# viodotcom/ppca_rs

Hardware: AMD Instinct MI355X
Metric: EM iters/sec (and samples/sec/iter) at N=10M d=256 k=10, 30% masked (higher is better)
Workload: dtype f64

## Files before the change

ppca_rs_amd/csrc/ppca_em9.hip:

```cpp
#include <cstdlib>

#include "ppca_device.hpp"

namespace ppca {

constexpr int E9_QW = 7;
constexpr int E9_F = 50;
constexpr int E9_HEAD = 6;
constexpr int E9_POISON = 100000;
constexpr int E9_EMIN = -900, E9_EMAX = 1000;
constexpr int E9_FLUSH_GROUPS = 100;
constexpr int E9_X_AUX = 2;
constexpr int E9_Q_AUX = 0;
constexpr int E9_LAC = 4;
constexpr int E9_HEAVY_BUDGET = 8;
constexpr int E9_GS_PAD = 18;
constexpr int E9_P4A_AHEAD = 1;

#ifdef PPCA_PHASE_TIMING
#define E9_FINE(i) { __builtin_amdgcn_sched_barrier(0); long long tn = clock64(); tfine[i] += tn - tfl; tfl = tn; __builtin_amdgcn_sched_barrier(0); }
#else
#define E9_FINE(i)
#endif

__device__ unsigned long long e9_counters[4];

template <int K>
struct Cfg9 {
    using c = Cfg<K>;
    static constexpr int KP = c::KP, NTP = c::NTP, B = c::B, DP = c::DP, XS = c::XS, CS = c::CS;
    static constexpr int NC = KP + K + 1;
    static constexpr int NCT = (NC + 15) / 16;
    static constexpr int NCOL = 16 * NCT;
    static constexpr int NCGB = (K + 3) / 4;
    static constexpr int NCL = NCGB < 2 ? NCGB : 2;
    static constexpr int PADC = K == 10 ? 14 : E9_GS_PAD;
    static constexpr int GS = 16 * NTP + PADC;
    static constexpr int WS = GS;
    static constexpr int NCP = NC;
    static constexpr int PLANE_BYTES = E9_QW * 2 * NCP * 16;
    static constexpr int OFF_X = 0;
    static constexpr int OFF_G = OFF_X + B * XS;
    static constexpr int OFF_W = OFF_G;
    static constexpr int OFF_M = OFF_G + 2 * B * GS;
    static constexpr int OFF_MB = OFF_M + 2 * B * 4;
    static constexpr int OFF_S = OFF_MB + DP * 2;
    static constexpr int OFF_L = OFF_S + 2 * B;
    static constexpr int OFF_P0 = OFF_L + 6 * B;
    static constexpr int OFF_P1 = OFF_P0 + PLANE_BYTES / 8;
    static constexpr int OFF_E = OFF_P1 + PLANE_BYTES / 8;
    static constexpr int OFF_BAR = OFF_E + NCOL / 2 + 4;
    static constexpr int OFF_K = OFF_BAR + 4;
    static constexpr int OFF_EB = OFF_K + 4;
    static constexpr int OFF_XT = OFF_EB + NCOL;
    static constexpr int OFF_CL = OFF_XT + 2 * B * 4;
    static constexpr int LDS_DOUBLES = OFF_CL + 2 * 16 * NCL * 32;
    static constexpr int p1slot(int a) { return a < PADC - K ? 16 * NTP + K + a : KP + (a - (PADC - K)); }
    static_assert(K - (PADC - K) <= 16 * NTP - KP, "free slots of a row hold the second partial of b");
    static_assert(NCOL / 2 <= 64, "one back wave digitises NCOL / 2 (column, chunk) items");
    static_assert(LDS_DOUBLES * 8 <= 160 * 1024, "LDS budget");
};

__device__ __forceinline__ void role_barrier(unsigned *ctr, unsigned &target, int lane) {
    asm volatile("s_waitcnt lgkmcnt(0)" ::: "memory");
    target += 4;
    if (lane == 0) __hip_atomic_fetch_add(ctr, 1u, __ATOMIC_RELAXED, __HIP_MEMORY_SCOPE_WORKGROUP);
    for (;;) {
        const unsigned seen = __builtin_amdgcn_readfirstlane(__hip_atomic_load(ctr, __ATOMIC_RELAXED, __HIP_MEMORY_SCOPE_WORKGROUP));
        if ((int)(seen - target) >= 0) break;
        __builtin_amdgcn_s_sleep(1);
    }
    asm volatile("" ::: "memory");
}
__device__ __forceinline__ void wait_counter(const unsigned *ctr, unsigned need) {
    for (;;) {
        const unsigned seen = __builtin_amdgcn_readfirstlane(__hip_atomic_load(ctr, __ATOMIC_RELAXED, __HIP_MEMORY_SCOPE_WORKGROUP));
        if ((int)(seen - need) >= 0) break;
        __builtin_amdgcn_s_sleep(1);
    }
    asm volatile("" ::: "memory");
}


template <int K, bool GATHER, bool WEIGHTED>
__global__ __launch_bounds__(512) void em9_kernel(PassArgs p) {
    using cfg = Cfg9<K>;
    constexpr int KP = cfg::KP, NTP = cfg::NTP, B = cfg::B, XS = cfg::XS, CS = cfg::CS, GS = cfg::GS,
                  WS = cfg::WS, NC = cfg::NC, NCT = cfg::NCT, NCOL = cfg::NCOL, NCP = cfg::NCP;
    constexpr int NF = 4;
    constexpr int RPW = B / NF;
    constexpr int DPS = cfg::DP / 2;
    constexpr int RT = 16 / NF;
    constexpr int DW = cfg::DP / NF;
    constexpr int QW = E9_QW;
    static_assert(NTP <= NF, "int8 Gram: one front wave per packed-column tile");
    static_assert(QS == 8, "digit grouping assumes 8 slices");
    extern __shared__ __attribute__((aligned(16))) double sm[];
    double *Xs = sm + cfg::OFF_X;
    double *Gs = sm + cfg::OFF_G;
    double *Ws = sm + cfg::OFF_W;
    unsigned long long *Ms = reinterpret_cast<unsigned long long *>(sm + cfg::OFF_M);
    unsigned *Mb = reinterpret_cast<unsigned *>(sm + cfg::OFF_MB);
    double *xxs = sm + cfg::OFF_S;
    double *scl = sm + cfg::OFF_L;
    int *Ex = reinterpret_cast<int *>(sm + cfg::OFF_E);
    unsigned *ctr = reinterpret_cast<unsigned *>(sm + cfg::OFF_BAR);
    unsigned *fbar = ctr, *bbar = ctr + 1, *digdone = ctr + 2, *vstamp = ctr + 3, *wready = ctr + 4, *itdone = ctr + 5, *cbar = ctr + 6;

    if (p.qflag) {
        int unsafe = 0;
#pragma unroll
        for (int t = 0; t < NTP; ++t) unsafe |= p.qflag[t];
        if (unsafe) return;
    }
    const int tid = threadIdx.x, lane_entry = tid & 63;
    const int wave8 = __builtin_amdgcn_readfirstlane(tid >> 6);
    const bool front = wave8 < NF;
    const int wave = wave8 & (NF - 1);
    const int d = p.d;
    const int64_t n = p.n_dev ? (int64_t)*p.n_dev : p.n;
    const double *mC = p.model + MODEL_HDR;
    const double *mMean = mC + (int64_t)d * K;
    const double s2_k = p.model[1], lnsig_k = p.model[2];

    constexpr bool PAIRS = K >= 2;
    constexpr int L_DEV = 0, L_LLK = L_DEV + B, L_W = L_DEV + 2 * B, L_NE = L_DEV + 3 * B, L_PM = L_DEV + 4 * B, L_PX = L_DEV + 5 * B;
    for (int idx = tid; idx < L_DEV + 6 * B; idx += 512) scl[idx] = (idx >= L_PM && idx < L_PX) ? 1.0 : 0.0;
    for (int idx = tid; idx < cfg::DP * 4; idx += 512) Mb[idx] = 0u;
    {
        constexpr int NCL = cfg::NCL, NCGB = cfg::NCGB;
        for (int idx = tid; idx < 2 * 16 * NCL * 32; idx += 512) {
            const int e = idx & 31, blk = idx >> 5, c = blk % NCL, hq = blk / NCL;
            sm[cfg::OFF_CL + idx] = p.cpb[(hq * NCGB + c) * 32 + e];
        }
    }
    if (tid < 8) ctr[tid] = 0u;
    if (tid < 4) Ex[NCOL + tid] = 0;
    if (tid < NCOL) sm[cfg::OFF_EB + tid] = 0.0;
    if (tid == 0) {
        sm[cfg::OFF_K] = s2_k;
        sm[cfg::OFF_K + 1] = 1.0 / s2_k;
        sm[cfg::OFF_K + 2] = lnsig_k;
    }

    const int64_t ntiles = (n + B - 1) / B;
    const int64_t tiles_per_wg = (ntiles + gridDim.x - 1) / gridDim.x;
    const int64_t tile_begin = (int64_t)blockIdx.x * tiles_per_wg;
    const int64_t tile_end = tile_begin + tiles_per_wg < ntiles ? tile_begin + tiles_per_wg : ntiles;
#ifdef PPCA_PHASE_TIMING
    long long tfine[16] = {0, 0, 0, 0, 0, 0, 0, 0, 0, 0, 0, 0, 0, 0, 0, 0};
    long long tfl = clock64();
#endif
    __syncthreads();

    if (!front) {
        typedef double acc_t;
        acc_t accM[RT][NCT][4];
#pragma unroll
        for (int r = 0; r < RT; ++r)
#pragma unroll
            for (int t = 0; t < NCT; ++t)
#pragma unroll
                for (int q = 0; q < 4; ++q) accM[r][t][q] = (acc_t)0;
        unsigned bbar_target = 0u;
        unsigned attempt = 0u;
        int pending = 0;
        int have_scale = 0, flushed = 0, groups = 0;
        int n_rescale = 0, n_flush = 0;
        int hbudget = E9_HEAVY_BUDGET;
        double *ebs = sm + cfg::OFF_EB;
        int rows_win = 0;
        unsigned char *smb = reinterpret_cast<unsigned char *>(sm);
        constexpr int P0_BYTES = cfg::OFF_P0 * 8, PG_BYTES = cfg::OFF_P1 * 8;
        StatsLayout L(d, K);
        double *out = p.part + (int64_t)blockIdx.x * L.len;

        const double *Wcur = Ws;
        auto wsrc = [&](int c) { return c < KP ? c : 16 * NTP + (c - KP); };

        auto digitise = [&](int lane, int dst_bytes, auto heavy_tag, unsigned heavy) -> bool {
            constexpr bool HEAVY = decltype(heavy_tag)::value;
            asm volatile("" : "+v"(lane));
            const bool active = lane < NCOL / 2;
            const int it = (NCOL / 2) * wave + (active ? lane : 0);
            const int c = it >> 1, chunk = it & 1;
            const unsigned hmine = HEAVY ? (heavy >> (16 * chunk)) & 0xFFFFu : 0u;
            const bool cvalid = c < NC;
            const int src = cvalid ? wsrc(c) : 0;
            const int E = Ex[c];
            const bool poisoned = E > 5000;
            const double qsc = __hiloint2double((1023 + E9_F - (poisoned ? 0 : E)) << 20, 0);
            const double magic = __hiloint2double(0x43388080, (int)0x80808080);
            unsigned bad = 0u;
            unsigned pl[QW][4];
            const double *wsrcp = Wcur + (16 * chunk) * WS + src;
#pragma unroll
            for (int g4 = 0; g4 < 4; ++g4) {
                unsigned wlo[4], whi[4];
#pragma unroll
                for (int j = 0; j < 4; ++j) {
                    const double wv = wsrcp[(4 * g4 + j) * WS];
                    const bool take = HEAVY ? cvalid && !((hmine >> (4 * g4 + j)) & 1u) : cvalid;
                    const double v = __builtin_fma(take ? wv : 0.0, qsc, magic);
                    const unsigned lo = (unsigned)__double2loint(v) ^ 0x80808080u;
                    const unsigned hi = (unsigned)__double2hiint(v) ^ 0x43388080u;
                    bad |= hi;
                    const int top = __builtin_amdgcn_sbfe((int)hi, 16, 4);
                    wlo[j] = lo;
                    whi[j] = __builtin_amdgcn_perm((unsigned)top, hi, 0x0C040100u);
                }
                auto tr4 = [&](const unsigned *w, unsigned *o0, unsigned *o1, unsigned *o2, unsigned *o3) {
                    const unsigned t0 = __builtin_amdgcn_perm(w[1], w[0], 0x05010400u), t1 = __builtin_amdgcn_perm(w[1], w[0], 0x07030602u);
                    const unsigned u0 = __builtin_amdgcn_perm(w[3], w[2], 0x05010400u), u1 = __builtin_amdgcn_perm(w[3], w[2], 0x07030602u);
                    *o0 = __builtin_amdgcn_perm(u0, t0, 0x05040100u);
                    *o1 = __builtin_amdgcn_perm(u0, t0, 0x07060302u);
                    *o2 = __builtin_amdgcn_perm(u1, t1, 0x05040100u);
                    if (o3) *o3 = __builtin_amdgcn_perm(u1, t1, 0x07060302u);
                };
                tr4(wlo, &pl[0][g4], &pl[1][g4], &pl[2][g4], &pl[3][g4]);
                tr4(whi, &pl[4][g4], &pl[5][g4], &pl[6][g4], nullptr);
                __builtin_amdgcn_sched_barrier(0);
            }
            if (active && cvalid) {
                unsigned char *wq = smb + dst_bytes;
#pragma unroll
                for (int sl = 0; sl < QW; ++sl)
                    *reinterpret_cast<i4_t *>(wq + ((sl * 2 + chunk) * NCP + c) * 16) =
                        i4_t{(int)pl[sl][0], (int)pl[sl][1], (int)pl[sl][2], (int)pl[sl][3]};
            }
            const bool mine = active && cvalid && !poisoned && (bad >> 20) != 0u;
            return __builtin_amdgcn_ballot_w64(mine) != 0ull;
        };

        auto rescale = [&](int lane, bool robust) {
            asm volatile("" : "+v"(lane));
            const bool active = lane < NCOL / 2;
            const int it = (NCOL / 2) * wave + (active ? lane : 0);
            const int c = it >> 1, chunk = it & 1;
            const bool cvalid = c < NC;
            const int src = cvalid ? wsrc(c) : 0;
            double m = 0.0;
            bool fin = true;
            if (!robust) {
#pragma unroll
                for (int j = 0; j < 16; ++j) {
                    const double av = __builtin_fabs(cvalid ? Wcur[(16 * chunk + j) * WS + src] : 0.0);
                    fin = fin && (av < __builtin_inf());
                    m = __builtin_fmax(m, av);
                }
            } else {
                const int hm = p.heavy_max;
                double cand = 0.0, mx = 0.0;
                for (int j = 0; j < 16; ++j) {
                    const double av = __builtin_fabs(cvalid ? Wcur[(16 * chunk + j) * WS + src] : 0.0);
                    fin = fin && (av < __builtin_inf());
                    mx = __builtin_fmax(mx, av);
                    int above = 0;
                    for (int i = 0; i < 32; ++i) above += __builtin_fabs(cvalid ? Wcur[i * WS + src] : 0.0) > av ? 1 : 0;
                    if (above >= hm) cand = __builtin_fmax(cand, av);
                }
                cand = __builtin_fmax(cand, dpp_f64<0xB1, 0xF>(cand));
                mx = __builtin_fmax(mx, dpp_f64<0xB1, 0xF>(mx));
                m = cand > 0.0 ? cand : mx;
            }
            m = __builtin_fmax(m, dpp_f64<0xB1, 0xF>(m));
            const int finw = __builtin_amdgcn_update_dpp(0, fin ? 1 : 0, 0xB1, 0xF, 0xF, true);
            fin = fin && finw != 0;
            const int Eold = have_scale ? Ex[c] : E9_EMIN;
            int Enew = Eold;
            if (m > 0.0) {
                int e = __builtin_amdgcn_frexp_exp(m) + E9_HEAD;
                e = e < E9_EMIN ? E9_EMIN : e;
                Enew = e > Eold ? e : Eold;
            }
            if (!fin || Enew > E9_EMAX) Enew = E9_POISON;
            if (Eold > 5000) Enew = Eold;
            if (active && chunk == 0) Ex[c] = Enew;
        };

        int *hvw = Ex + NCOL;
        auto heavy_bits = [&](int lane) {
            asm volatile("" : "+v"(lane));
            const bool active = lane < NCOL / 2;
            const int it = (NCOL / 2) * wave + (active ? lane : 0);
            const int c = it >> 1, chunk = it & 1;
            const bool cvalid = c < NC;
            const int src = cvalid ? wsrc(c) : 0;
            const int E = Ex[c];
            const bool live = active && cvalid && E <= 5000;
            const double qsc = __hiloint2double((1023 + E9_F - (live ? E : 0)) << 20, 0);
            const double magic = __hiloint2double(0x43388080, (int)0x80808080);
            unsigned bits = 0u, nogo = 0u;
            for (int j = 0; j < 16; ++j) {
                const double wv = live ? Wcur[(16 * chunk + j) * WS + src] : 0.0;
                const double v = __builtin_fma(wv, qsc, magic);
                const unsigned hi = (unsigned)__double2hiint(v) ^ 0x43388080u;
                if ((hi >> 20) != 0u) {
                    bits |= 1u << (16 * chunk + j);
                    if (!(__builtin_fabs(wv) < __builtin_inf()) || __builtin_amdgcn_frexp_exp(wv) + E9_F - E > 1000) nogo = 1u;
                }
            }
            if (bits) __hip_atomic_fetch_or(reinterpret_cast<unsigned *>(hvw), bits, __ATOMIC_RELAXED, __HIP_MEMORY_SCOPE_WORKGROUP);
            if (nogo) __hip_atomic_fetch_or(reinterpret_cast<unsigned *>(hvw + 1), 1u, __ATOMIC_RELAXED, __HIP_MEMORY_SCOPE_WORKGROUP);
        };
        auto heavy_add = [&](int lane, unsigned hv, int slot) {
            asm volatile("" : "+v"(lane));
            const int l15 = lane & 15, l4 = lane >> 4;
            unsigned mw[RT][4];
#pragma unroll
            for (int r = 0; r < RT; ++r)
#pragma unroll
                for (int q = 0; q < 4; ++q) mw[r][q] = Mb[(DW * wave + 16 * r + 4 * l4 + q) * 4 + slot];
            double sc[NCT];
            int src[NCT];
#pragma unroll
            for (int t = 0; t < NCT; ++t) {
                const int c = 16 * t + l15;
                const int E = Ex[c];
                sc[t] = (c < NC && E <= 5000) ? __hiloint2double((1023 + E9_F - E) << 20, 0) : 0.0;
                src[t] = c < NC ? wsrc(c) : 0;
            }
            for (unsigned rest = hv; rest != 0u; rest &= rest - 1u) {
                const int i = __builtin_ctz(rest);
                const int bitpos = 8 * (i >> 3) + 7 - (i & 7);
                double wv[NCT];
#pragma unroll
                for (int t = 0; t < NCT; ++t) wv[t] = Wcur[i * WS + src[t]] * sc[t];
#pragma unroll
                for (int r = 0; r < RT; ++r)
#pragma unroll
                    for (int q = 0; q < 4; ++q) {
                        const bool obs = (mw[r][q] >> bitpos) & 1u;
#pragma unroll
                        for (int t = 0; t < NCT; ++t) accM[r][t][q] += obs ? wv[t] : 0.0;
                    }
            }
        };

        auto emit = [&](int lane, bool accumulate, bool clear) {
            asm volatile("" : "+v"(lane));
            const int l15 = lane & 15, l4 = lane >> 4;
            const double win = 4.0 * __builtin_sqrt((double)rows_win);
            rows_win = 0;
#pragma unroll
            for (int t = 0; t < NCT; ++t) {
                const int c = 16 * t + l15, a = c - KP;
                const int E = have_scale ? Ex[c] : 0;
                if (wave == 0 && l4 == 0 && have_scale && E <= 5000) ebs[c] += win * __hiloint2double((1023 + E - E9_F) << 20, 0);
                const double fsc = __hiloint2double(E > 5000 ? 0x7FF80000 : (1023 + E - E9_F) << 20, 0);
#pragma unroll
                for (int r = 0; r < RT; ++r)
#pragma unroll
                    for (int q = 0; q < 4; ++q) {
                        const int dim = DW * wave + 16 * r + 4 * l4 + q;
                        double v = have_scale ? (double)accM[r][t][q] * fsc : 0.0;
                        if (E > 5000) v = fsc;
                        if (clear) accM[r][t][q] = (acc_t)0;
                        if (dim < d && c < NC) {
                            double *dst = c < KP ? out + L.S + (int64_t)dim * KP + c
                                                 : (a < K ? out + L.U + (int64_t)dim * K + a : out + L.totals + dim);
                            *dst = accumulate ? *dst + v : v;
                        }
                    }
            }
        };

        auto contract = [&](int lane, bool both, int slot_first, int slot_second) {
            asm volatile("" : "+v"(lane));
            const int l15 = lane & 15, l4 = lane >> 4, lh = l4 >> 1;
            i4_t af[RT];
#pragma unroll
            for (int r = 0; r < RT; ++r) {
                const unsigned word = Mb[(DW * wave + 16 * r + l15) * 4 + (lh ? slot_second : slot_first)];
                unsigned f = (word >> (16 * (l4 & 1))) & 0xFFFFu;
                f = (both || lh == 0) ? f : 0u;
                const unsigned g = __builtin_bitreverse32(f);
                af[r][0] = (int)((((g >> 24) & 0xFu) * 0x00204081u) & 0x01010101u);
                af[r][1] = (int)((((g >> 28) & 0xFu) * 0x00204081u) & 0x01010101u);
                af[r][2] = (int)((((g >> 16) & 0xFu) * 0x00204081u) & 0x01010101u);
                af[r][3] = (int)((((g >> 20) & 0xFu) * 0x00204081u) & 0x01010101u);
            }
            const unsigned char *wq = smb + (lh == 0 ? P0_BYTES : PG_BYTES) + ((l4 & 1) * NCP + l15) * 16;
            constexpr int PSTRIDE = 2 * NCP * 16;
            constexpr int NBLK = NCT * 3 * RT;
            i4_t dd[2][3];
            i4_t bb[3];
            auto issue = [&](auto i_tag) {
                constexpr int i = decltype(i_tag)::value, t = i / (3 * RT), batch = (i / RT) % 3, r = i % RT;
                const unsigned char *wt = wq + t * 256 + 3 * batch * PSTRIDE;
                if constexpr (r == 0) {
                    bb[0] = *reinterpret_cast<const i4_t *>(wt);
                    if constexpr (batch < 2) {
                        bb[1] = *reinterpret_cast<const i4_t *>(wt + PSTRIDE);
                        bb[2] = *reinterpret_cast<const i4_t *>(wt + 2 * PSTRIDE);
                    }
                }
                if constexpr (batch < 2) mfma_i8_x3(af[r], bb[0], bb[1], bb[2], dd[i & 1][0], dd[i & 1][1], dd[i & 1][2]);
                else mfma_i8_x1(af[r], bb[0], dd[i & 1][0]);
            };
            auto fold = [&](auto i_tag) {
                constexpr int i = decltype(i_tag)::value, t = i / (3 * RT), batch = (i / RT) % 3, r = i % RT;
                const i4_t *d3 = dd[i & 1];
#pragma unroll
                for (int q = 0; q < 4; ++q) {
                    if constexpr (batch < 2) {
                        int pc;
                        asm("v_lshl_add_u32 %0, %1, 8, %2" : "=v"(pc) : "v"(d3[2][q]), "v"(d3[1][q]));
                        asm("v_lshl_add_u32 %0, %1, 8, %2" : "=v"(pc) : "v"(pc), "v"(d3[0][q]));
                        if constexpr (batch == 0) accM[r][t][q] += (double)pc;
                        else accM[r][t][q] = __builtin_fma((double)pc, 0x1p24, accM[r][t][q]);
                    } else {
                        accM[r][t][q] = __builtin_fma((double)d3[0][q], 0x1p48, accM[r][t][q]);
                    }
                }
            };
            issue(std::integral_constant<int, 0>{});
            static_for<NBLK>([&](auto i_tag) {
                constexpr int i = decltype(i_tag)::value;
                if constexpr (i + 1 < NBLK) issue(std::integral_constant<int, i + 1>{});
                fold(i_tag);
            });
        };

        for (int64_t tile = tile_begin; tile < tile_end; ++tile) {
            int lane = lane_entry;
            asm volatile("" : "+v"(lane));
            const int rel = (int)(tile - tile_begin);
            const bool last = tile + 1 == tile_end;
            const int slot_cur = rel & 3, slot_prev = (rel + 3) & 3;
            Wcur = Ws + (rel & 1) * B * WS;
            wait_counter(wready, 4u * (unsigned)(rel + 1));
#pragma unroll 1
            for (;;) {
                ++attempt;
                const bool bad = !have_scale || digitise(lane, pending ? PG_BYTES : P0_BYTES, std::false_type{}, 0u);
                if (bad && lane == 0) __hip_atomic_store(vstamp, attempt, __ATOMIC_RELAXED, __HIP_MEMORY_SCOPE_WORKGROUP);
                role_barrier(bbar, bbar_target, lane_entry);
                bool viol = __builtin_amdgcn_readfirstlane(__hip_atomic_load(vstamp, __ATOMIC_RELAXED, __HIP_MEMORY_SCOPE_WORKGROUP)) == attempt;
                bool hv_dirty = false;
                if (viol && have_scale && p.heavy_max > 0) {
                    heavy_bits(lane);
                    role_barrier(bbar, bbar_target, lane_entry);
                    const unsigned hv = (unsigned)__builtin_amdgcn_readfirstlane(__hip_atomic_load(hvw, __ATOMIC_RELAXED, __HIP_MEMORY_SCOPE_WORKGROUP));
                    const unsigned nogo = (unsigned)__builtin_amdgcn_readfirstlane(__hip_atomic_load(hvw + 1, __ATOMIC_RELAXED, __HIP_MEMORY_SCOPE_WORKGROUP));
                    hv_dirty = true;
                    if (hv != 0u && nogo == 0u && __builtin_popcount(hv) <= p.heavy_max && hbudget > 0) {
                        --hbudget;
                        (void)digitise(lane, pending ? PG_BYTES : P0_BYTES, std::true_type{}, hv);
                        heavy_add(lane, hv, slot_cur);
                        role_barrier(bbar, bbar_target, lane_entry);
                        if (wave == 0 && lane_entry < 2) hvw[lane_entry] = 0;
                        hv_dirty = false;
                        viol = false;
                    }
                }
                if (!viol) {
                    if (lane_entry == 0) __hip_atomic_fetch_add(digdone, 1u, __ATOMIC_RELAXED, __HIP_MEMORY_SCOPE_WORKGROUP);
                    rows_win += B;
                }
                const bool con = pending || (!viol && last);
                if (con) {
                    contract(lane, !viol && pending, pending ? slot_prev : slot_cur, slot_cur);
                    ++groups;
                }
                pending = (!viol && !con) ? 1 : 0;
                if (viol ? have_scale != 0 : groups >= E9_FLUSH_GROUPS) {
                    emit(lane, flushed != 0, true);
                    flushed = 1;
                    groups = 0;
                    n_flush += viol ? 0 : 1;
                    if (!viol) hbudget = E9_HEAVY_BUDGET;
                }
                if (!viol) break;
                n_rescale += have_scale;
                role_barrier(bbar, bbar_target, lane_entry);
                if (hv_dirty && wave == 0 && lane_entry < 2) hvw[lane_entry] = 0;
                rescale(lane, !have_scale && p.heavy_max > 0);
                have_scale = 1;
                role_barrier(bbar, bbar_target, lane_entry);
            }
            asm volatile("s_waitcnt lgkmcnt(0)" ::: "memory");
            if (lane_entry == 0) __hip_atomic_fetch_add(itdone, 1u, __ATOMIC_RELAXED, __HIP_MEMORY_SCOPE_WORKGROUP);
        }
        emit(lane_entry, flushed != 0, false);
        if (p.errb && wave == 0 && lane_entry < 16) {
#pragma unroll
            for (int t = 0; t < NCT; ++t) p.errb[(int64_t)blockIdx.x * W_GUARD_NCOL + 16 * t + lane_entry] = ebs[16 * t + lane_entry];
        }
        if (tid == 256) {
            if (n_rescale) atomicAdd(&e9_counters[0], (unsigned long long)n_rescale);
            if (n_flush) atomicAdd(&e9_counters[1], (unsigned long long)n_flush);
            atomicMax(&e9_counters[2], (unsigned long long)(tile_end > tile_begin ? tile_end - tile_begin : 0));
            if (blockIdx.x == 0) atomicAdd(&e9_counters[3], 1ull);
        }
        return;
    }

    unsigned fbar_target = 0u;
    constexpr int NCG = (K + 1 + 3) / 4;
    double accX[RT][NCG];
#pragma unroll
    for (int r = 0; r < RT; ++r)
#pragma unroll
        for (int c = 0; c < NCG; ++c) accX[r][c] = 0.0;
    const double inv_s2_k = 1.0 / s2_k;
    double xr[RPW][4];
    const int64_t nleft = n - tile_begin * B;
    const int nrel = (int)(nleft < (1 << 30) ? nleft : (1 << 30));
    const double *Xwg = p.X + tile_begin * B * p.ldx;
    const int64_t own = (tile_end - tile_begin) * B;
    const int nmine = tile_end > tile_begin ? (int)(own < nleft ? own : nleft) : 0;
    const int *rows_wg = (GATHER && p.rows) ? p.rows + tile_begin * B : nullptr;
    const int rowbytes = d * (int)sizeof(double);
    auto tile_rsrc = [&](int64_t tile) {
        const int rel0 = (int)(tile - tile_begin) * B;
        int cnt = nrel - rel0;
        cnt = __builtin_amdgcn_readfirstlane(cnt < 0 ? 0 : (cnt > B ? B : cnt));
        return __builtin_amdgcn_make_buffer_rsrc(const_cast<double *>(Xwg + (int64_t)rel0 * p.ldx), 0, cnt * rowbytes, 0x00020000);
    };
    int gidx = 0;
    double gw = 0.0;
    auto fetch_meta = [&](int64_t tile) {
        const int rel = (int)(tile - tile_begin) * B + wave * RPW + (lane_entry & (RPW - 1));
        const int rc = rel < nrel ? rel : nrel - 1;
        if constexpr (GATHER) {
            if (rows_wg) gidx = rows_wg[rc];
        }
        if constexpr (WEIGHTED) gw = p.w[tile_begin * B + rc];
    };
    auto load_row = [&](const __amdgpu_buffer_rsrc_t &trs, int64_t tile, int r) {
        typedef unsigned u4_t __attribute__((ext_vector_type(4)));
        if constexpr (GATHER) {
            if (rows_wg) {
                const int rel = (int)(tile - tile_begin) * B + wave * RPW + r;
                const int rc = rel < nrel ? rel : nrel - 1;
                const __amdgpu_buffer_rsrc_t xrsrc = __builtin_amdgcn_make_buffer_rsrc(
                    const_cast<double *>(p.X + (int64_t)__builtin_amdgcn_readlane(gidx, r) * p.ldx), 0, rc < 0 ? 0 : rowbytes, 0x00020000);
#pragma unroll
                for (int h = 0; h < 2; ++h) {
                    const u4_t v = __builtin_amdgcn_raw_buffer_load_b128(xrsrc, lane_entry * 16, 1024 * h, E9_X_AUX);
                    xr[r][2 * h] = __longlong_as_double(((long long)v[1] << 32) | v[0]);
                    xr[r][2 * h + 1] = __longlong_as_double(((long long)v[3] << 32) | v[2]);
                }
                return;
            }
        }
#pragma unroll
        for (int h = 0; h < 2; ++h) {
            const u4_t v = __builtin_amdgcn_raw_buffer_load_b128(trs, lane_entry * 16, (wave * RPW + r) * rowbytes + 1024 * h, E9_X_AUX);
            xr[r][2 * h] = __longlong_as_double(((long long)v[1] << 32) | v[0]);
            xr[r][2 * h + 1] = __longlong_as_double(((long long)v[3] << 32) | v[2]);
        }
    };
    const __amdgpu_buffer_rsrc_t qrsrc = __builtin_amdgcn_make_buffer_rsrc(p.qtab, 0, (int)qtab_bytes<K>(), 0x00020000);
    const bool gram_wave = NTP >= NF || wave < NTP;
    i4_t qbA[2][4];
    i4_t qbB[2][4];
    auto load_pair = [&](i4_t(&dst)[2][4], int sl0) {
        int qbase = wave * QS * 4 * 1024;
        asm volatile("" : "+s"(qbase));
#pragma unroll
        for (int u = 0; u < 2; ++u)
#pragma unroll
            for (int kc = 0; kc < 4; ++kc) {
                typedef unsigned u4_t __attribute__((ext_vector_type(4)));
                const u4_t v = __builtin_amdgcn_raw_buffer_load_b128(qrsrc, lane_entry * 16 + kc * 1024, qbase + (sl0 + u) * 4096, E9_Q_AUX);
                dst[u][kc] = i4_t{(int)v[0], (int)v[1], (int)v[2], (int)v[3]};
            }
    };
    double mu[4], lim[4];
    int st_wlo = 0, st_whi = 0;
    int st_mb[4] = {0, 0, 0, 0};
    double xx_run = 0.0;
    double sq_run = 0.0;
    double muq[4] = {0.0, 0.0, 0.0, 0.0};
    auto load_mu = [&]() {
        const __amdgpu_buffer_rsrc_t mrs = __builtin_amdgcn_make_buffer_rsrc(const_cast<double *>(mMean), 0, d * (int)sizeof(double), 0x00020000);
#pragma unroll
        for (int q = 0; q < 4; ++q) {
            typedef unsigned u2_t __attribute__((ext_vector_type(2)));
            const u2_t v2 = __builtin_amdgcn_raw_buffer_load_b64(mrs, lane_entry * 16 + 8 * (q & 1), 1024 * (q >> 1), 0);
            muq[q] = __longlong_as_double(((long long)v2[1] << 32) | v2[0]);
        }
    };
    auto stage_row = [&](int64_t t, int lane, auto r_tag) {
        constexpr int r = decltype(r_tag)::value;
        const int ri = wave * RPW + r;
        double pc_xx = 0.0;
        static_for<2>([&](auto h_tag) {
            constexpr int h = decltype(h_tag)::value;
            double xt[2];
            unsigned long long bal[2];
#pragma unroll
            for (int e = 0; e < 2; ++e) {
                const double v = xr[r][2 * h + e];
                const bool ob = __builtin_fabs(v) < lim[2 * h + e];
                bal[e] = __builtin_amdgcn_ballot_w64(ob);
                xt[e] = ob ? v - mu[2 * h + e] : 0.0;
            }
            file_mask<4 * r + 2 * h>(st_wlo, st_whi, st_mb[2 * h], bal[0]);
            file_mask<4 * r + 2 * h + 1>(st_wlo, st_whi, st_mb[2 * h + 1], bal[1]);
            typedef double d2_t __attribute__((ext_vector_type(2)));
            *reinterpret_cast<d2_t *>(Xs + ri * XS + 128 * h + 2 * lane) = d2_t{xt[0], xt[1]};
            pc_xx += xt[0] * xt[0];
            pc_xx += xt[1] * xt[1];
        });
        const bool mine = (int)(t - tile_begin) * B + ri < nmine;
        double wr = 1.0;
        if constexpr (WEIGHTED) {
            const long long gb = __double_as_longlong(gw);
            const int lo = __builtin_amdgcn_readlane((int)gb, r), hi = __builtin_amdgcn_readlane((int)(gb >> 32), r);
            wr = __longlong_as_double(((long long)hi << 32) | (unsigned)lo);
        }
        wr = mine ? wr : 0.0;
        xx_run += wr * pc_xx;
    };
    auto stage_tile = [&](int64_t t, int lane) {
        {
            mu[0] = muq[0]; mu[1] = muq[1]; mu[2] = muq[2]; mu[3] = muq[3];
#pragma unroll
            for (int q = 0; q < 4; ++q) lim[q] = (128 * (q >> 1) + 2 * lane + (q & 1) < d) ? __builtin_inf() : -1.0;
        }
        const int rel = (int)(t - tile_begin);
        st_wlo = st_whi = 0;
        st_mb[0] = st_mb[1] = st_mb[2] = st_mb[3] = 0;
        static_for<RPW>([&](auto r_tag) { stage_row(t, lane, r_tag); });
        const unsigned long long myw = ((unsigned long long)(unsigned)st_whi << 32) | (unsigned)st_wlo;
        if (lane < 4 * RPW) Ms[(rel & 1) * 4 * B + wave * 4 * RPW + lane] = myw;
        unsigned char *mbb = reinterpret_cast<unsigned char *>(Mb);
        const int slot = rel & 3;
#pragma unroll
        for (int q = 0; q < 4; ++q)
            mbb[(128 * (q >> 1) + 2 * lane + (q & 1)) * 16 + 4 * slot + wave] = (unsigned char)st_mb[q];
    };

    if (tile_begin < tile_end) {
        const __amdgpu_buffer_rsrc_t trs = tile_rsrc(tile_begin);
        if constexpr (GATHER || WEIGHTED) fetch_meta(tile_begin);
#pragma unroll
        for (int r = 0; r < RPW; ++r) load_row(trs, tile_begin, r);
        load_mu();
        load_pair(qbA, 6);
        load_pair(qbB, 4);
        stage_tile(tile_begin, lane_entry);
        if constexpr (GATHER || WEIGHTED) fetch_meta(tile_begin + 1);
    }
    role_barrier(fbar, fbar_target, lane_entry);

    constexpr int LPER = (16 * NTP) / 32;
    constexpr bool LMAJ = (16 * NTP) % 32 == 0 && B == 32 && (KP + (LPER > 0 ? LPER : 1) - 1) / (LPER > 0 ? LPER : 1) + 2 <= B;
    constexpr int LROWS = LMAJ ? (KP + LPER - 1) / LPER : 0;
    constexpr int PADC = cfg::PADC, ZIN = PADC - K - 1;
    auto zslot = [](int a, int i) {
        if (a < ZIN) return i * GS + 16 * NTP + K + 1 + a;
        a -= ZIN;
        if (LMAJ) return (LROWS + a / (LPER > 0 ? LPER : 1)) * GS + (a % (LPER > 0 ? LPER : 1)) * 32 + i;
        return i * GS + KP + a;
    };
    static_assert(!LMAJ || LROWS + (K - ZIN > 0 ? (K - ZIN + LPER - 1) / (LPER > 0 ? LPER : 1) : 0) <= B, "entry-major z rows");
    static_assert(ZIN >= 0 && (LMAJ || ZIN + (16 * NTP - KP) >= K), "free slots of a row hold z");

    auto lslot = [](int e, int i) { return LMAJ ? (e / (LPER > 0 ? LPER : 1)) * GS + (e % (LPER > 0 ? LPER : 1)) * 32 + i : i * GS + e; };

    for (int64_t tile = tile_begin; tile <= tile_end; ++tile) {
        int lane = lane_entry;
        asm volatile("" : "+v"(lane));
        const int l15 = lane & 15, l4 = lane >> 4;
        const int colb = (l15 < K) ? l15 : K;
        const int rel = (int)(tile - tile_begin);
        const bool cur = tile < tile_end;
        const unsigned long long *Msc = Ms + (rel & 1) * 4 * B;
        double *Gcur = Gs + (rel & 1) * B * GS;
        double *Gprev = Gs + ((rel + 1) & 1) * B * GS;
        if (cur) {
            const int rt = wave & 1, kq = wave >> 1;
            constexpr int NCGB = (K + 3) / 4;
            double bsum[NCGB];
            const unsigned dd_early = __hip_atomic_load(digdone, __ATOMIC_RELAXED, __HIP_MEMORY_SCOPE_WORKGROUP);
            i4_t af[2][4];
            double v[2][4];
            auto group = [&](const i4_t(*qb)[4], bool first) {
#pragma unroll
                for (int rt2 = 0; rt2 < 2; ++rt2) {
                    i4_t ia[2];
#pragma unroll
                    for (int u = 0; u < 2; ++u) {
                        ia[u] = i4_t{0, 0, 0, 0};
#pragma unroll
                        for (int kc = 0; kc < 4; ++kc)
                            ia[u] = __builtin_amdgcn_mfma_i32_16x16x64_i8(af[rt2][kc], qb[u][kc], ia[u], 0, 0, 0);
                    }
#pragma unroll
                    for (int r = 0; r < 4; ++r) {
                        const int part = ia[1][r] * QBASE + ia[0][r];
                        v[rt2][r] = first ? (double)part : v[rt2][r] * (double)(QBASE * QBASE) + (double)part;
                    }
                }
            };
                constexpr int NQ = DPS / 8;
                constexpr int LAC = E9_LAC, LAX = 2;
                const int j4 = lane & 3, sb = (lane >> 2) & 1, kb = (lane >> 3) & 1;
                const double *xrow = Xs + (16 * rt + 4 * sb + j4) * XS + DPS * kq + 16 * kb + l4;
                const __amdgpu_buffer_rsrc_t crs =
                    __builtin_amdgcn_make_buffer_rsrc(const_cast<double *>(p.cpb), 0, CPB_DOUBLES * (int)sizeof(double), 0x00020000);
                const int cvo = ((2 * l4 + kb) * 4 + j4) * 8;
                constexpr int NSO = (NQ * NCGB * 256 + 4095) / 4096;
                int cso[NSO];
#pragma unroll
                for (int u = 0; u < NSO; ++u) {
                    cso[u] = kq * (NQ * NCGB * 256) + 4096 * u;
                    asm volatile("" : "+s"(cso[u]));
                }
                double accb[NCGB][2];
#pragma unroll
                for (int c = 0; c < NCGB; ++c) accb[c][0] = accb[c][1] = 0.0;
                double cb[LAC + 1][NCGB], xb[LAX + 1][2];
                constexpr int NCLc = cfg::NCL;
                const double *clp = sm + cfg::OFF_CL + kq * (NQ * NCLc * 32) + (2 * l4 + kb) * 4 + j4;
                auto cload_lds = [&](auto q_tag) {
                    constexpr int q = decltype(q_tag)::value;
#pragma unroll
                    for (int c = 0; c < NCLc; ++c) cb[q % (LAC + 1)][c] = clp[(q * NCLc + c) * 32];
                };
                auto cload = [&](auto q_tag) {
                    constexpr int q = decltype(q_tag)::value;
#pragma unroll
                    for (int c = NCLc; c < NCGB; ++c) {
                        typedef unsigned u2_t __attribute__((ext_vector_type(2)));
                        const int off = (q * NCGB + c) * 256;
                        const u2_t v2 = __builtin_amdgcn_raw_buffer_load_b64(crs, cvo + (off & 4095), cso[off >> 12], 0);
                        cb[q % (LAC + 1)][c] = __longlong_as_double(((long long)v2[1] << 32) | v2[0]);
                    }
                };
                auto xload = [&](auto q_tag) {
                    constexpr int q = decltype(q_tag)::value;
#pragma unroll
                    for (int g = 0; g < 2; ++g) xb[q % (LAX + 1)][g] = xrow[8 * g * XS + 32 * (q >> 2) + 4 * (q & 3)];
                };
            double qs = 0.0;
            {
                unsigned long long mwd[2][4];
#pragma unroll
                for (int rt2 = 0; rt2 < 2; ++rt2)
#pragma unroll
                    for (int kc = 0; kc < 4; ++kc) mwd[rt2][kc] = Msc[(16 * rt2 + l15) * 4 + kc];
                __builtin_amdgcn_sched_barrier(0);
                if (gram_wave) qs = p.qscale[16 * wave + l15];
                static_for<LAC>([&](auto q_tag) { cload(q_tag); });
                __builtin_amdgcn_sched_barrier(0);
#pragma unroll
                for (int rt2 = 0; rt2 < 2; ++rt2)
#pragma unroll
                    for (int kc = 0; kc < 4; ++kc) {
                        const unsigned bits = (unsigned)(mwd[rt2][kc] >> (16 * l4)) & 0xFFFFu;
#pragma unroll
                        for (int u = 0; u < 4; ++u)
                            af[rt2][kc][u] = (int)((((bits >> (4 * u)) & 0xFu) * 0x00204081u) & 0x01010101u);
                    }
                group(qbA, true);
                load_pair(qbA, 2);
                group(qbB, false);
                load_pair(qbB, 0);
            }
            E9_FINE(15)
            {
                static_for<LAX>([&](auto q_tag) {
                    xload(q_tag);
                    cload_lds(q_tag);
                });
                static_for<NQ>([&](auto q_tag) {
                    constexpr int q = decltype(q_tag)::value;
                    if constexpr (q + LAC < NQ) cload(std::integral_constant<int, q + LAC>{});
                    if constexpr (q + LAX < NQ) {
                        xload(std::integral_constant<int, q + LAX>{});
                        cload_lds(std::integral_constant<int, q + LAX>{});
                    }
                    __builtin_amdgcn_sched_barrier(0);
#pragma unroll
                    for (int c = 0; c < NCGB; ++c)
#pragma unroll
                        for (int g = 0; g < 2; ++g)
                            accb[c][g] = __builtin_amdgcn_mfma_f64_4x4x4f64(cb[q % (LAC + 1)][c], xb[q % (LAX + 1)][g], accb[c][g], 0, 0, 0);
                    __builtin_amdgcn_sched_barrier(0);
                });
#pragma unroll
                for (int c = 0; c < NCGB; ++c) {
                    const double t0 = accb[c][0] + dpp_f64<0x128, 0xF>(accb[c][0]);
                    const double t1 = accb[c][1] + dpp_f64<0x128, 0xF>(accb[c][1]);
                    bsum[c] = kb ? t1 : t0;
                }
            }
            E9_FINE(4)
            group(qbA, false);
            group(qbB, false);
            E9_FINE(0)
            const unsigned need_dd = rel >= 2 ? 4u * (unsigned)(rel - 1) : 0u;
            if ((int)((unsigned)__builtin_amdgcn_readfirstlane(dd_early) - need_dd) < 0) wait_counter(digdone, need_dd);
            E9_FINE(1)
            if (gram_wave) {
#pragma unroll
                for (int rt2 = 0; rt2 < 2; ++rt2)
#pragma unroll
                    for (int r = 0; r < 4; ++r)
                        if (16 * wave + l15 < KP) Gcur[(16 * rt2 + 4 * l4 + r) * GS + 16 * wave + l15] = v[rt2][r] * qs;
            }
#pragma unroll
            for (int c = 0; c < NCGB; ++c) {
                const int a = 4 * c + l4;
                if (a < K) Gcur[(16 * rt + l15) * GS + (kq == 0 ? 16 * NTP + a : cfg::p1slot(a))] = bsum[c];
            }
        }
        E9_FINE(2)
        role_barrier(fbar, fbar_target, lane_entry);
        E9_FINE(3)
        const int solver = rel & (NF - 1);
        constexpr int SCAL_UNITS = 107;
        if (PAIRS || lane < B) {
            const double s2 = sm[cfg::OFF_K], inv_s2 = sm[cfg::OFF_K + 1], lnsig = sm[cfg::OFF_K + 2];
            const int i = lane & (B - 1);
            const int hi = PAIRS ? lane >> 5 : 0;
            double sc_sq = 0.0;
            if (wave == solver) {
                if (cur) {
                    const int64_t row = tile * B + i;
                    double *g0 = Gcur + i * GS;
                    const double wgt = (row < n) ? (WEIGHTED ? p.w[row] : 1.0) : 0.0;
                    const int m = __popcll(Msc[i * 4]) + __popcll(Msc[i * 4 + 1]) + __popcll(Msc[i * 4 + 2]) + __popcll(Msc[i * 4 + 3]);
                    Posterior<K> fac;
                    double pm = 1.0;
                    int pe = 0;
                    double z[K], quad = 0.0, zz = 0.0;
                    fac.load([&](int e) { return g0[e]; }, s2);
#pragma unroll
                    for (int a = 0; a < K; ++a) z[a] = g0[16 * NTP + a] + g0[cfg::p1slot(a)];
                    E9_FINE(7)
                    fac.factor_loaded(pm, pe);
                    E9_FINE(9)
                    fac.solve_loaded(z, quad, zz);
                    E9_FINE(10)
                    if (hi == 0) {
#pragma unroll
                        for (int e = 0; e < KP; ++e) Gcur[lslot(e, i)] = fac.L[e];
#pragma unroll
                        for (int a = 0; a < K; ++a) Gcur[zslot(a, i)] = z[a];
#pragma unroll
                        for (int a = 0; a < K; ++a) g0[16 * NTP + a] = wgt * z[a];
                        g0[16 * NTP + K] = wgt;
                        double *xt = sm + cfg::OFF_XT + ((rel & 1) * B + i) * 4;
                        xt[0] = quad;
                        xt[1] = zz;
                        xt[2] = pm;
                        xt[3] = (double)pe;
                    }
                }
            } else if (rel > 0) {
                const int cw = (wave - solver - 1) & (NF - 1);
                const int64_t row = (tile - 1) * B + i;
                double *wrow = Gprev + i * GS;
                const double wgt = (row < n) ? (WEIGHTED ? p.w[row] : 1.0) : 0.0;
                const unsigned long long *Msp = Ms + ((rel + 1) & 1) * 4 * B;
                const int m = __popcll(Msp[i * 4]) + __popcll(Msp[i * 4 + 1]) + __popcll(Msp[i * 4 + 2]) + __popcll(Msp[i * 4 + 3]);
                Posterior<K> post;
                double z[K];
#pragma unroll
                for (int e = 0; e < KP; ++e) post.L[e] = Gprev[lslot(e, i)];
#pragma unroll
                for (int a = 0; a < K; ++a) z[a] = Gprev[zslot(a, i)];
                asm volatile("s_waitcnt lgkmcnt(0)" ::: "memory");
                if (lane_entry == 0) __hip_atomic_fetch_add(cbar, 1u, __ATOMIC_RELAXED, __HIP_MEMORY_SCOPE_WORKGROUP);
                wait_counter(cbar, 3u * (unsigned)rel);
                double trpart = 0.0;
                if constexpr (PAIRS) {
#pragma unroll
                    for (int pp = 0; pp < (K + 1) / 2; ++pp) {
                        if (pair_owner_eq(K, pp, NF - 1, SCAL_UNITS) != cw) continue;
                        const int c0 = 2 * pp;
                        const double zc = (hi && c0 + 1 < K) ? z[c0 + 1 < K ? c0 + 1 : c0] : z[c0];
                        trpart += post.minv_column_pair(c0, hi, [&](int t, double v, bool ok) {
                            if (ok && c0 + hi < K) wrow[tri(t, c0) + hi] = wgt * (z[t] * zc + s2 * v);
                        });
                    }
                } else {
#pragma unroll
                    for (int c = 0; c < K; ++c) {
                        if (column_owner_eq(K, c, NF - 1, SCAL_UNITS) != cw) continue;
                        trpart += post.minv_column(c, [&](int a, int cc, double v) { wrow[tri(a, cc)] = wgt * (z[a] * z[cc] + s2 * v); });
                    }
                }
                if (m > 0) sc_sq -= wgt * s2 * s2 * trpart;
                if (cw == NF - 2 && hi == 0) {
                    const double *xt = sm + cfg::OFF_XT + (((rel + 1) & 1) * B + i) * 4;
                    const double quad = xt[0], zz = xt[1], pm = xt[2];
                    const int pe = (int)xt[3];
                    double sc_dev = 0.0, sc_llk = 0.0, sc_w = 0.0, sc_ne = 0.0;
                    const double run_dev = scl[L_DEV + i], run_llk = scl[L_LLK + i], run_w = scl[L_W + i], run_ne = scl[L_NE + i];
                    const double run_pm = scl[L_PM + i], run_px = scl[L_PX + i];
                    if (m > 0) {
                        sc_sq += wgt * s2 * (double)K;
                        sc_dev += wgt * (0.0 - quad - s2 * zz);
                        sc_ne += (row < n) ? 1.0 : 0.0;
                    }
                    const double lk0 = sample_llk_nolog(0.0, quad, inv_s2, lnsig, m, K);
                    if constexpr (WEIGHTED) {
                        if (!p.no_llk) sc_llk += wgt * (m > 0 ? lk0 - 0.5 * Posterior<K>::logdet(pm, pe) : 0.0);
                    } else {
                        const bool use = m > 0 && row < n;
                        sc_llk += use ? lk0 : 0.0;
                        int e;
                        scl[L_PM + i] = frexp(run_pm * (use ? pm : 1.0), &e);
                        scl[L_PX + i] = run_px + (double)(e + (use ? pe : 0));
                    }
                    sc_w += wgt;
                    scl[L_DEV + i] = run_dev + sc_dev;
                    scl[L_LLK + i] = run_llk + sc_llk;
                    scl[L_W + i] = run_w + sc_w;
                    scl[L_NE + i] = run_ne + sc_ne;
                }
            }
            sq_run += sc_sq;
        }
        if (wave == solver) { E9_FINE(6) } else { E9_FINE(8) }
        role_barrier(fbar, fbar_target, lane_entry);
        E9_FINE(5)
        if (rel > 0 && lane_entry == 0) __hip_atomic_fetch_add(wready, 1u, __ATOMIC_RELAXED, __HIP_MEMORY_SCOPE_WORKGROUP);
        if (!cur) break;
        {
            load_pair(qbA, 6);
            load_mu();
            load_pair(qbB, 4);
            constexpr int AH = E9_P4A_AHEAD, NB3 = AH + 1;
            double bzb[NB3][NCG], axb[NB3][RT];
            const __amdgpu_buffer_rsrc_t trs = tile_rsrc(tile + 1);
            const int j4 = lane & 3;
#pragma unroll
            for (int s0 = 0; s0 < AH; ++s0) {
                const int smp = 4 * s0 + l4;
#pragma unroll
                for (int c = 0; c < NCG; ++c) bzb[s0][c] = Gcur[smp * WS + 16 * NTP + 4 * c + j4];
#pragma unroll
                for (int r = 0; r < RT; ++r) axb[s0][r] = Xs[smp * XS + DW * wave + 16 * r + l15];
            }
#pragma unroll
            for (int s = 0; s < 8; ++s) {
                if (s < RPW) load_row(trs, tile + 1, s);
                if (s + AH < 8) {
                    const int smp = 4 * (s + AH) + l4;
#pragma unroll
                    for (int c = 0; c < NCG; ++c) bzb[(s + AH) % NB3][c] = Gcur[smp * WS + 16 * NTP + 4 * c + j4];
#pragma unroll
                    for (int r = 0; r < RT; ++r) axb[(s + AH) % NB3][r] = Xs[smp * XS + DW * wave + 16 * r + l15];
                }
                __builtin_amdgcn_sched_barrier(0);
#pragma unroll
                for (int r = 0; r < RT; ++r)
#pragma unroll
                    for (int c = 0; c < NCG; ++c)
                        accX[r][c] = __builtin_amdgcn_mfma_f64_4x4x4f64(axb[s % NB3][r], bzb[s % NB3][c], accX[r][c], 0, 0, 0);
                __builtin_amdgcn_sched_barrier(0);
            }
        }
        E9_FINE(11)
        role_barrier(fbar, fbar_target, lane_entry);
        E9_FINE(12)
        if (rel >= 2) wait_counter(itdone, 4u * (unsigned)(rel - 1));
        stage_tile(tile + 1, lane);
        if constexpr (GATHER || WEIGHTED) fetch_meta(tile + 2);
        E9_FINE(13)
        role_barrier(fbar, fbar_target, lane_entry);
        E9_FINE(14)
    }
#ifdef PPCA_PHASE_TIMING
    if (p.dbg && lane_entry == 0)
        for (int i = 0; i < 16; ++i) p.dbg[(int64_t)gridDim.x * 16 + ((int64_t)blockIdx.x * 8 + wave8) * 16 + i] = (double)tfine[i];
#endif

    {
        const int lane = lane_entry, l15 = lane & 15, l4 = lane >> 4;
        const double sq_w = wave_sum(sq_run);
        const double xx_w = wave_sum(xx_run);
        if (lane == 0) {
            xxs[wave] = sq_w;
            xxs[NF + wave] = xx_w;
        }
        role_barrier(fbar, fbar_target, lane_entry);
        StatsLayout L(d, K);
        double *out = p.part + (int64_t)blockIdx.x * L.len;
        if (wave == 0) {
            double v0 = 0.0, xx_tot = 0.0;
#pragma unroll
            for (int w = 0; w < NF; ++w) v0 += xxs[w];
#pragma unroll
            for (int w = 0; w < NF; ++w) xx_tot += xxs[NF + w];
            const int li = lane < B ? lane : 0;
            double sc_llk = scl[L_LLK + li];
            if constexpr (!WEIGHTED) sc_llk -= 0.5 * (log(scl[L_PM + li]) + scl[L_PX + li] * LN_2);
            const double v1 = wave_sum(lane < B ? scl[L_DEV + li] : 0.0), v2 = wave_sum(lane < B ? sc_llk : 0.0),
                         v3 = wave_sum(lane < B ? scl[L_W + li] : 0.0), v4 = wave_sum(lane < B ? scl[L_NE + li] : 0.0);
            if (lane == 0) {
                double *sc = out + L.scalars;
                sc[SC_SQERR] = v0;
                sc[SC_DEVSQ] = v1 + xx_tot;
                sc[SC_LLK] = v2 - 0.5 * inv_s2_k * xx_tot;
                sc[SC_SUMW] = v3;
                sc[SC_NONEMPTY] = v4;
                sc[5] = 0.0;
                sc[6] = 0.0;
                sc[7] = 0.0;
            }
        }
#pragma unroll
        for (int r = 0; r < RT; ++r) {
            const int dim = DW * wave + 16 * r + 4 * ((lane >> 2) & 3) + l4;
            if (dim >= d) continue;
#pragma unroll
            for (int c = 0; c < NCG; ++c) {
                const int col = 4 * c + (lane & 3);
                if (col < K) out[L.cross + (int64_t)dim * K + col] = accX[r][c];
                else if (col == K) out[L.sumx + dim] = accX[r][c];
            }
        }
    }
}

template <int K, bool GATHER, bool WEIGHTED>
static hipError_t launch_em9_t(int grid, const PassArgs &a, hipStream_t s) {
    const size_t lds = sizeof(double) * Cfg9<K>::LDS_DOUBLES;
    if (hipError_t e = ensure_dynamic_lds<em9_kernel<K, GATHER, WEIGHTED>>(lds); e != hipSuccess) return e;
    hipLaunchKernelGGL((em9_kernel<K, GATHER, WEIGHTED>), dim3(grid), dim3(512), lds, s, a);
    return hipGetLastError();
}

hipError_t em9_debug_counters(unsigned long long *out4, int reset, hipStream_t s) {
    if (hipError_t e = hipMemcpyFromSymbolAsync(out4, HIP_SYMBOL(e9_counters), sizeof(unsigned long long) * 4, 0, hipMemcpyDeviceToHost, s);
        e != hipSuccess)
        return e;
    if (hipError_t e = hipStreamSynchronize(s); e != hipSuccess) return e;
    if (reset) {
        const unsigned long long z[4] = {0, 0, 0, 0};
        if (hipError_t e = hipMemcpyToSymbolAsync(HIP_SYMBOL(e9_counters), z, sizeof(z), 0, hipMemcpyHostToDevice, s); e != hipSuccess) return e;
        return hipStreamSynchronize(s);
    }
    return hipSuccess;
}

bool em9_covers(int k) {
#ifdef PPCA_DEV_K10
    return k == 10;
#else
    return k >= 1 && k <= FUSED_MAX_K;
#endif
}

hipError_t launch_em9(int k, int grid, const PassArgs &a, hipStream_t s) {
    const bool gather = a.rows != nullptr;
#define PPCA_E9_CASE(KK) \
    case KK:             \
        return gather ? launch_em9_t<KK, true, true>(grid, a, s) : (a.w ? launch_em9_t<KK, false, true>(grid, a, s) : launch_em9_t<KK, false, false>(grid, a, s));
    switch (k) {
#ifdef PPCA_DEV_K10
        PPCA_E9_CASE(10)
#else
        PPCA_E9_CASE(1) PPCA_E9_CASE(2) PPCA_E9_CASE(3) PPCA_E9_CASE(4) PPCA_E9_CASE(5) PPCA_E9_CASE(6) PPCA_E9_CASE(7)
        PPCA_E9_CASE(8) PPCA_E9_CASE(9) PPCA_E9_CASE(10)
#endif
        default: return hipErrorInvalidValue;
    }
#undef PPCA_E9_CASE
}

}
```

Measured before the change: 104.2.

## Pack partial tail column tile's int8 digit planes into one MFMA tile

When the number of Gram columns leaves a partial last 16-column tile, the seven int8 digit slices of those tail columns are packed side by side into a single 16-wide tile. The Gram MFMA stage then needs one tile's worth of MFMAs for the tail instead of three slice batches. Digitisation is split into 8-sample chunks, with the tail digitised by a rotating wave. Emit recombines the per-slice partial sums with lane shuffles scaled by 256. This cuts MFMA count and LDS plane size for K=10, at the cost of extra shuffle recombination and a more intricate plane layout.

```diff
diff --git a/ppca_rs_amd/csrc/ppca_em9.hip b/ppca_rs_amd/csrc/ppca_em9.hip
--- a/ppca_rs_amd/csrc/ppca_em9.hip
+++ b/ppca_rs_amd/csrc/ppca_em9.hip
@@ -37,8 +37,14 @@
     static constexpr int PADC = K == 10 ? 14 : E9_GS_PAD;
     static constexpr int GS = 16 * NTP + PADC;
     static constexpr int WS = GS;
-    static constexpr int NCP = NC;
-    static constexpr int PLANE_BYTES = E9_QW * 2 * NCP * 16;
+    static constexpr int NT = NC % 16;
+    static constexpr bool PACK_TAIL = NT != 0 && E9_QW * NT <= 16;
+    static constexpr int NMAIN = PACK_TAIL ? NC - NT : NC;
+    static constexpr int NMT = (NMAIN + 15) / 16;
+    static constexpr int TAILP = E9_QW * NT;
+    static constexpr int NCP = NMAIN;
+    static constexpr int MAIN_BYTES = E9_QW * 2 * NCP * 16;
+    static constexpr int PLANE_BYTES = MAIN_BYTES + (PACK_TAIL ? 2 * TAILP * 16 : 0);
     static constexpr int OFF_X = 0;
     static constexpr int OFF_G = OFF_X + B * XS;
     static constexpr int OFF_W = OFF_G;
@@ -57,7 +63,9 @@
     static constexpr int LDS_DOUBLES = OFF_CL + 2 * 16 * NCL * 32;
     static constexpr int p1slot(int a) { return a < PADC - K ? 16 * NTP + K + a : KP + (a - (PADC - K)); }
     static_assert(K - (PADC - K) <= 16 * NTP - KP, "free slots of a row hold the second partial of b");
-    static_assert(NCOL / 2 <= 64, "one back wave digitises NCOL / 2 (column, chunk) items");
+    static_assert(16 * NMT <= 64, "one back wave digitises one (column, 8-sample chunk) item per lane: 16 NMT lanes");
+    static_assert(NCOL / 2 <= 64, "rescale / heavy_bits: one back wave scans NCOL / 2 (column, 16-sample chunk) items");
+    static_assert(!PACK_TAIL || (NMAIN % 16 == 0 && 4 * NT <= 64 && PLANE_BYTES % 16 == 0), "packed tail tile");
     static_assert(LDS_DOUBLES * 8 <= 160 * 1024, "LDS budget");
 };
 
@@ -86,7 +94,9 @@
 __global__ __launch_bounds__(512) void em9_kernel(PassArgs p) {
     using cfg = Cfg9<K>;
     constexpr int KP = cfg::KP, NTP = cfg::NTP, B = cfg::B, XS = cfg::XS, CS = cfg::CS, GS = cfg::GS,
-                  WS = cfg::WS, NC = cfg::NC, NCT = cfg::NCT, NCOL = cfg::NCOL, NCP = cfg::NCP;
+                  WS = cfg::WS, NC = cfg::NC, NCT = cfg::NCT, NCOL = cfg::NCOL, NCP = cfg::NCP, NT = cfg::NT, NMAIN = cfg::NMAIN,
+                  NMT = cfg::NMT, TAILP = cfg::TAILP, MAIN_BYTES = cfg::MAIN_BYTES;
+    constexpr bool PACK_TAIL = cfg::PACK_TAIL;
     constexpr int NF = 4;
     constexpr int RPW = B / NF;
     constexpr int DPS = cfg::DP / 2;
@@ -178,24 +188,25 @@
         const double *Wcur = Ws;
         auto wsrc = [&](int c) { return c < KP ? c : 16 * NTP + (c - KP); };
 
-        auto digitise = [&](int lane, int dst_bytes, auto heavy_tag, unsigned heavy) -> bool {
-            constexpr bool HEAVY = decltype(heavy_tag)::value;
+        int tail_wave = 0;
+        auto cut8 = [&](int lane, int dst_bytes, auto heavy_tag, unsigned heavy, auto tail_tag) -> bool {
+            constexpr bool HEAVY = decltype(heavy_tag)::value, TAIL = decltype(tail_tag)::value;
             asm volatile("" : "+v"(lane));
-            const bool active = lane < NCOL / 2;
-            const int it = (NCOL / 2) * wave + (active ? lane : 0);
-            const int c = it >> 1, chunk = it & 1;
-            const unsigned hmine = HEAVY ? (heavy >> (16 * chunk)) & 0xFFFFu : 0u;
-            const bool cvalid = c < NC;
+            const bool active = lane < (TAIL ? 4 * NT : 16 * NMT);
+            const int it = TAIL ? (active ? lane : 0) : 16 * NMT * wave + (active ? lane : 0);
+            const int c = TAIL ? NMAIN + (it >> 2) : 16 * (it >> 6) + (it & 15), ch8 = TAIL ? it & 3 : (it >> 4) & 3;
+            const unsigned hmine = HEAVY ? (heavy >> (8 * ch8)) & 0xFFu : 0u;
+            const bool cvalid = TAIL || c < NMAIN;
             const int src = cvalid ? wsrc(c) : 0;
             const int E = Ex[c];
             const bool poisoned = E > 5000;
             const double qsc = __hiloint2double((1023 + E9_F - (poisoned ? 0 : E)) << 20, 0);
             const double magic = __hiloint2double(0x43388080, (int)0x80808080);
             unsigned bad = 0u;
-            unsigned pl[QW][4];
-            const double *wsrcp = Wcur + (16 * chunk) * WS + src;
-#pragma unroll
-            for (int g4 = 0; g4 < 4; ++g4) {
+            unsigned pl[QW][2];
+            const double *wsrcp = Wcur + (8 * ch8) * WS + src;
+#pragma unroll
+            for (int g4 = 0; g4 < 2; ++g4) {
                 unsigned wlo[4], whi[4];
 #pragma unroll
                 for (int j = 0; j < 4; ++j) {
@@ -222,13 +233,21 @@
                 __builtin_amdgcn_sched_barrier(0);
             }
             if (active && cvalid) {
-                unsigned char *wq = smb + dst_bytes;
-#pragma unroll
-                for (int sl = 0; sl < QW; ++sl)
-                    *reinterpret_cast<i4_t *>(wq + ((sl * 2 + chunk) * NCP + c) * 16) =
-                        i4_t{(int)pl[sl][0], (int)pl[sl][1], (int)pl[sl][2], (int)pl[sl][3]};
-            }
-            const bool mine = active && cvalid && !poisoned && (bad >> 20) != 0u;
+                typedef int i2_t __attribute__((ext_vector_type(2)));
+                unsigned char *wq = smb + dst_bytes + 8 * (ch8 & 1);
+#pragma unroll
+                for (int sl = 0; sl < QW; ++sl) {
+                    const int row = TAIL ? (ch8 >> 1) * TAILP + QW * (c - NMAIN) + sl : (sl * 2 + (ch8 >> 1)) * NCP + c;
+                    *reinterpret_cast<i2_t *>(wq + (TAIL ? MAIN_BYTES : 0) + row * 16) = i2_t{(int)pl[sl][0], (int)pl[sl][1]};
+                }
+            }
+            return active && cvalid && !poisoned && (bad >> 20) != 0u;
+        };
+        auto digitise = [&](int lane, int dst_bytes, auto heavy_tag, unsigned heavy) -> bool {
+            bool mine = cut8(lane, dst_bytes, heavy_tag, heavy, std::false_type{});
+            if constexpr (PACK_TAIL) {
+                if (wave == tail_wave) mine = cut8(lane, dst_bytes, heavy_tag, heavy, std::true_type{}) || mine;
+            }
             return __builtin_amdgcn_ballot_w64(mine) != 0ull;
         };
 
@@ -315,7 +334,8 @@
             int src[NCT];
 #pragma unroll
             for (int t = 0; t < NCT; ++t) {
-                const int c = 16 * t + l15;
+                const bool tail = PACK_TAIL && t == NCT - 1;
+                const int c = tail ? (l15 % QW == 0 && l15 < TAILP ? NMAIN + l15 / QW : NCOL - 1) : 16 * t + l15;
                 const int E = Ex[c];
                 sc[t] = (c < NC && E <= 5000) ? __hiloint2double((1023 + E9_F - E) << 20, 0) : 0.0;
                 src[t] = c < NC ? wsrc(c) : 0;
@@ -325,7 +345,7 @@
                 const int bitpos = 8 * (i >> 3) + 7 - (i & 7);
                 double wv[NCT];
 #pragma unroll
-                for (int t = 0; t < NCT; ++t) wv[t] = Wcur[i * WS + src[t]] * sc[t];
+                for (int t = 0; t < NCT; ++t) wv[t] = sc[t] != 0.0 ? Wcur[i * WS + src[t]] * sc[t] : 0.0;
 #pragma unroll
                 for (int r = 0; r < RT; ++r)
 #pragma unroll
@@ -344,19 +364,32 @@
             rows_win = 0;
 #pragma unroll
             for (int t = 0; t < NCT; ++t) {
-                const int c = 16 * t + l15, a = c - KP;
+                const bool tail = PACK_TAIL && t == NCT - 1;
+                const int tj = l15 < TAILP ? l15 / QW : NT - 1;
+                const bool owner = !tail || (l15 < TAILP && l15 == QW * tj);
+                const int c = tail ? NMAIN + tj : 16 * t + l15, a = c - KP;
                 const int E = have_scale ? Ex[c] : 0;
-                if (wave == 0 && l4 == 0 && have_scale && E <= 5000) ebs[c] += win * __hiloint2double((1023 + E - E9_F) << 20, 0);
+                if (wave == 0 && l4 == 0 && owner && have_scale && E <= 5000) ebs[c] += win * __hiloint2double((1023 + E - E9_F) << 20, 0);
                 const double fsc = __hiloint2double(E > 5000 ? 0x7FF80000 : (1023 + E - E9_F) << 20, 0);
 #pragma unroll
                 for (int r = 0; r < RT; ++r)
 #pragma unroll
                     for (int q = 0; q < 4; ++q) {
                         const int dim = DW * wave + 16 * r + 4 * l4 + q;
-                        double v = have_scale ? (double)accM[r][t][q] * fsc : 0.0;
+                        double av = (double)accM[r][t][q];
+                        if (tail) {
+                            double h = av;
+#pragma unroll
+                            for (int s = 1; s < QW; ++s) {
+                                const double up = __shfl(h, lane + 1, 64);
+                                h = (l15 - QW * tj == QW - 1 - s) ? __builtin_fma(up, 256.0, av) : h;
+                            }
+                            av = h;
+                        }
+                        double v = have_scale ? av * fsc : 0.0;
                         if (E > 5000) v = fsc;
                         if (clear) accM[r][t][q] = (acc_t)0;
-                        if (dim < d && c < NC) {
+                        if (dim < d && c < NC && owner) {
                             double *dst = c < KP ? out + L.S + (int64_t)dim * KP + c
                                                  : (a < K ? out + L.U + (int64_t)dim * K + a : out + L.totals + dim);
                             *dst = accumulate ? *dst + v : v;
@@ -382,11 +415,19 @@
             }
             const unsigned char *wq = smb + (lh == 0 ? P0_BYTES : PG_BYTES) + ((l4 & 1) * NCP + l15) * 16;
             constexpr int PSTRIDE = 2 * NCP * 16;
-            constexpr int NBLK = NCT * 3 * RT;
+            constexpr int NMBLK = NMT * 3 * RT;
+            constexpr int NBLK = NMBLK + (PACK_TAIL ? RT : 0);
+            static_assert(NMT + (PACK_TAIL ? 1 : 0) == NCT, "column tiles: the planes' and the packed tail");
             i4_t dd[2][3];
             i4_t bb[3];
             auto issue = [&](auto i_tag) {
                 constexpr int i = decltype(i_tag)::value, t = i / (3 * RT), batch = (i / RT) % 3, r = i % RT;
+                if constexpr (i >= NMBLK) {
+                    if constexpr (i == NMBLK)
+                        bb[0] = *reinterpret_cast<const i4_t *>(wq + MAIN_BYTES - ((lane_entry >> 4) & 1) * ((NCP - TAILP) * 16));
+                    mfma_i8_x1(af[i - NMBLK], bb[0], dd[i & 1][0]);
+                    return;
+                }
                 const unsigned char *wt = wq + t * 256 + 3 * batch * PSTRIDE;
                 if constexpr (r == 0) {
                     bb[0] = *reinterpret_cast<const i4_t *>(wt);
@@ -401,6 +442,11 @@
             auto fold = [&](auto i_tag) {
                 constexpr int i = decltype(i_tag)::value, t = i / (3 * RT), batch = (i / RT) % 3, r = i % RT;
                 const i4_t *d3 = dd[i & 1];
+                if constexpr (i >= NMBLK) {
+#pragma unroll
+                    for (int q = 0; q < 4; ++q) accM[i - NMBLK][NCT - 1][q] += (double)d3[0][q];
+                    return;
+                }
 #pragma unroll
                 for (int q = 0; q < 4; ++q) {
                     if constexpr (batch < 2) {
@@ -422,13 +468,14 @@
             });
         };
 
-        for (int64_t tile = tile_begin; tile < tile_end; ++tile) {
+        const int ntile_wg = __builtin_amdgcn_readfirstlane(tile_end > tile_begin ? (int)(tile_end - tile_begin) : 0);
+        for (int rel = 0; rel < ntile_wg; ++rel) {
             int lane = lane_entry;
             asm volatile("" : "+v"(lane));
-            const int rel = (int)(tile - tile_begin);
-            const bool last = tile + 1 == tile_end;
+            const bool last = rel + 1 == ntile_wg;
             const int slot_cur = rel & 3, slot_prev = (rel + 3) & 3;
             Wcur = Ws + (rel & 1) * B * WS;
+            tail_wave = rel & (NF - 1);
             wait_counter(wready, 4u * (unsigned)(rel + 1));
 #pragma unroll 1
             for (;;) {
@@ -490,7 +537,7 @@
         if (tid == 256) {
             if (n_rescale) atomicAdd(&e9_counters[0], (unsigned long long)n_rescale);
             if (n_flush) atomicAdd(&e9_counters[1], (unsigned long long)n_flush);
-            atomicMax(&e9_counters[2], (unsigned long long)(tile_end > tile_begin ? tile_end - tile_begin : 0));
+            atomicMax(&e9_counters[2], (unsigned long long)ntile_wg);
             if (blockIdx.x == 0) atomicAdd(&e9_counters[3], 1ull);
         }
         return;
```

Result: no change. 105.2, median of 6 (+0.9%).
